# joeyee/Onet

Hardware: AMD Instinct MI355X
Metric: training images/sec (twin 256x256 pass) (higher is better)
Workload: dtype f32

## Files before the change

### onet_amd/csrc/bn.hip

```cpp
#include <type_traits>
#include "common.hpp"

using namespace onet;

__global__ __launch_bounds__(256) void bn_stats_partial_kernel(const float* __restrict__ z, int64_t z_bs,
                                                               float* __restrict__ part, int C, int HW,
                                                               int chunks, int chunk_len) {
    __shared__ double red[16];
    const int c = blockIdx.x % C;
    const int p = blockIdx.x / C;
    const int b = p / chunks, ch = p % chunks;
    const float* src = z + (int64_t)b * z_bs + (int64_t)c * HW;
    const int beg = ch * chunk_len;
    const int end = min(beg + chunk_len, HW);
    const bool vec = ((HW & 3) == 0) && ((z_bs & 3) == 0) && ((chunk_len & 3) == 0);
    const double pivot = (double)src[beg];
    double v[2] = {0.0, 0.0};
    if (vec) {
        int i = beg + threadIdx.x * 4;
        for (; i + 3072 < end; i += 4096) {
            float4 q[4];
#pragma unroll
            for (int k = 0; k < 4; ++k) q[k] = *reinterpret_cast<const float4*>(src + i + 1024 * k);
#pragma unroll
// ... 563 lines not shown
    const float* ds = da + (int64_t)b * da_bs + (int64_t)c * HW;
    const int beg = ch * chunk_len, end = min(beg + chunk_len, HW);
    double v[2] = {0.0, 0.0};
    if (((HW & 3) == 0) && ((z_bs & 3) == 0) && ((da_bs & 3) == 0) && ((chunk_len & 3) == 0)) {
        int i = beg + threadIdx.x * 4;
        for (; i + 3072 < end; i += 4096) {
            float4 q[4], g[4];
#pragma unroll
            for (int k = 0; k < 4; ++k) {
                q[k] = bn_ldz4<ZT>(zs + i + 1024 * k);
                g[k] = *reinterpret_cast<const float4*>(ds + i + 1024 * k);
            }
#pragma unroll
            for (int k = 0; k < 4; ++k) {
                const float zz[4] = {q[k].x, q[k].y, q[k].z, q[k].w}, gg[4] = {g[k].x, g[k].y, g[k].z, g[k].w};
#pragma unroll
                for (int e = 0; e < 4; ++e) {
                    const double dy = fmaf(zz[e] - mean, sc, sh) > 0.f ? (double)gg[e] : 0.0;
                    v[0] += dy;
                    v[1] += dy * (((double)zz[e] - meand) * invd);
                    vmax = fmaxf(vmax, fabsf(gg[e]));
                }
            }
        }
        for (; i < end; i += 1024) {
            const float4 q = bn_ldz4<ZT>(zs + i);
            const float4 g = *reinterpret_cast<const float4*>(ds + i);
            const float zz[4] = {q.x, q.y, q.z, q.w}, gg[4] = {g.x, g.y, g.z, g.w};
#pragma unroll
            for (int k = 0; k < 4; ++k) {
                const double dy = fmaf(zz[k] - mean, sc, sh) > 0.f ? (double)gg[k] : 0.0;
                v[0] += dy;
                v[1] += dy * (((double)zz[k] - meand) * invd);
                vmax = fmaxf(vmax, fabsf(gg[k]));
            }
        }
    } else {
        for (int i = beg + threadIdx.x; i < end; i += 256) {
            const float zi = bn_ldz<ZT>(zs + i);
            const double dy = fmaf(zi - mean, sc, sh) > 0.f ? (double)ds[i] : 0.0;
            v[0] += dy;
            v[1] += dy * (((double)zi - meand) * invd);
            vmax = fmaxf(vmax, fabsf(ds[i]));
        }
    }
    amax_commit(vmax, amax);
    block_sum_256<double, 2>(v, red);
    if (threadIdx.x == 0) {
        float* o = part2 + ((int64_t)p * C + c) * 4;
        o[0] = (float)v[0];
        o[1] = (float)(v[0] - (double)o[0]);
        o[2] = (float)v[1];
        o[3] = (float)(v[1] - (double)o[2]);
    }
}

__global__ __launch_bounds__(256) void head_bwd_reduce_kernel(const float* __restrict__ L, int64_t L_bs, const float* __restrict__ z,
                                                              int64_t z_bs, const float* __restrict__ g, const float* __restrict__ at_t,
                                                              const float* __restrict__ at_d, const float* __restrict__ save,
                                                              float* __restrict__ dL, float* __restrict__ part2, int C, int HW, int chunks,
                                                              int chunk_len, unsigned* __restrict__ amax, int gimg) {
    __shared__ double red[8];
    float vmax = 0.f;
    const int c = blockIdx.x % C;
    const int p = blockIdx.x / C;
    const int b = p / chunks, ch = p % chunks;
    save += (int64_t)(b / gimg) * 4 * C;
    const float mean = save[c], invstd = save[C + c], sc = save[2 * C + c], sh = save[3 * C + c];
    const double meand = mean, invd = invstd;
    const float* zs = z + (int64_t)b * z_bs + (int64_t)c * HW;
    const float* ls = L + (int64_t)b * L_bs + (int64_t)c * HW;
    const float* gs = g + (int64_t)b * HW;
    const float* as = b < gimg ? at_t : at_d;
    if (as) as += (int64_t)(b % gimg) * HW;
    float* os = dL + ((int64_t)b * C + c) * HW;
    const int beg = ch * chunk_len, end = min(beg + chunk_len, HW);
    const float4 zero4 = make_float4(0.f, 0.f, 0.f, 0.f);
    double v[2] = {0.0, 0.0};
    auto four = [&](const float4& q, const float4& l, const float4& gv, const float4& av) -> float4 {
        const float zz[4] = {q.x, q.y, q.z, q.w}, ll[4] = {l.x, l.y, l.z, l.w}, gg[4] = {gv.x, gv.y, gv.z, gv.w}, aa[4] = {av.x, av.y, av.z, av.w};
        float o[4];
#pragma unroll
        for (int e = 0; e < 4; ++e) {
            const float x = fmaf(zz[e] - mean, sc, sh);
            o[e] = fmaf(gg[e], fmaxf(x, 0.f), aa[e]);
            const float da = gg[e] * ll[e];
            const double dy = x > 0.f ? (double)da : 0.0;
            v[0] += dy;
            v[1] += dy * (((double)zz[e] - meand) * invd);
            vmax = fmaxf(vmax, fabsf(da));
        }
        return make_float4(o[0], o[1], o[2], o[3]);
    };
    int i = beg + threadIdx.x * 4;
    for (; i + 3072 < end; i += 4096) {
        float4 q[4], l[4], gv[4], av[4];
#pragma unroll
        for (int k = 0; k < 4; ++k) {
            q[k] = *reinterpret_cast<const float4*>(zs + i + 1024 * k);
            l[k] = *reinterpret_cast<const float4*>(ls + i + 1024 * k);
            gv[k] = *reinterpret_cast<const float4*>(gs + i + 1024 * k);
            av[k] = as ? *reinterpret_cast<const float4*>(as + i + 1024 * k) : zero4;
        }
#pragma unroll
        for (int k = 0; k < 4; ++k) *reinterpret_cast<float4*>(os + i + 1024 * k) = four(q[k], l[k], gv[k], av[k]);
    }
// ... 197 lines not shown
}

int onet_bn_finalize_cm(const float* part, int nparts, int64_t c_stride, const float* gamma, const float* beta, float* running_mean,
                            float* running_var, float momentum, float eps, float* save, void* act_amax, int groups, int C, void* stream) {
    ONET_REQUIRE(part && save && nparts > 0 && C > 0 && groups >= 1 && c_stride >= (int64_t)nparts * groups * 3, "bn_finalize_cm: bad args");
    hipLaunchKernelGGL(bn_finalize_cm_kernel, dim3(C), dim3(256), 0, as_stream(stream), part, nparts, c_stride, gamma, beta, running_mean,
                       running_var, momentum, eps, save, C, (unsigned*)act_amax, groups);
    return check_launch("bn_finalize_cm_kernel");
}

int onet_bn_eval_coeffs(const float* gamma, const float* beta, const float* running_mean,
                        const float* running_var, float eps, float* save, int C, void* stream) {
    ONET_REQUIRE(running_mean && running_var && save && C > 0, "bn_eval_coeffs: bad args");
    hipLaunchKernelGGL(bn_eval_coeffs_kernel, dim3(cdiv(C, 256)), dim3(256), 0, as_stream(stream), gamma, beta,
                       running_mean, running_var, eps, save, C);
    return check_launch("bn_eval_coeffs_kernel");
}

int onet_bn_relu_apply(const void* z, int z_bf16, int64_t z_bs, float* a, int64_t a_bs, const float* save, void* amax, int group_images,
                            int B, int C, int HW, void* stream) {
    ONET_REQUIRE(z && a && save && B > 0 && C > 0 && HW > 0 && group_images >= 0, "bn_relu_apply: bad args");
    const int chunks = cdiv(HW, 4096);
    const int64_t blocks = (int64_t)B * C * chunks;
    ONET_REQUIRE(blocks < (1ll << 31), "bn_relu_apply: grid too large");
    if (z_bf16) {
        ONET_REQUIRE((reinterpret_cast<uintptr_t>(z) & 7) == 0, "bn_relu_apply: 8-byte aligned bf16 rows required");
        hipLaunchKernelGGL(bn_relu_apply_kernel<__bf16>, dim3((unsigned)blocks), dim3(256), 0, as_stream(stream), (const __bf16*)z, z_bs, a, a_bs,
                           save, C, HW, chunks, (unsigned*)amax, group_images);
    } else {
        hipLaunchKernelGGL(bn_relu_apply_kernel<float>, dim3((unsigned)blocks), dim3(256), 0, as_stream(stream), (const float*)z, z_bs, a, a_bs,
                           save, C, HW, chunks, (unsigned*)amax, group_images);
    }
    return check_launch("bn_relu_apply_kernel");
}

int onet_bn_relu_apply_pool(const float* z, int64_t z_bs, float* a, int64_t a_bs, float* y, int64_t y_bs, const float* save,
                                 void* amax, int B, int C, int H, int W, void* stream) {
    ONET_REQUIRE(z && a && y && save && B > 0 && C > 0 && H > 0 && W > 0, "bn_relu_apply_pool: bad args");
    auto al = [](const void* p, uintptr_t m) { return (reinterpret_cast<uintptr_t>(p) & m) == 0; };
    if ((H & 1) || (W & 3) || (z_bs & 3) || (a_bs & 3) || (y_bs & 1) || !al(z, 15) || !al(a, 15) || !al(y, 7)) return 1;
    const int npatch = (H / 2) * (W / 4), bpp = cdiv(npatch, 256);
    const int64_t blocks = (int64_t)B * C * bpp;
    ONET_REQUIRE(blocks < (1ll << 31), "bn_relu_apply_pool: grid too large");
    hipLaunchKernelGGL(bn_relu_apply_pool_kernel, dim3((unsigned)blocks), dim3(256), 0, as_stream(stream), z, z_bs, a, a_bs,
                       y, y_bs, save, C, H, W, bpp, (unsigned*)amax);
    return check_launch("bn_relu_apply_pool_kernel");
}

int onet_bn_relu_bwd_reduce(const float* da, int64_t da_bs, const void* z, int z_bf16, int64_t z_bs, const float* save, float* part2,
                                 int nparts, void* da_amax, int group_images, int B, int C, int HW, void* stream) {
    ONET_REQUIRE(da && z && save && part2 && B > 0 && C > 0 && HW > 0 && group_images >= 0, "bn_relu_bwd_reduce: bad args");
    int chunks, chunk_len;
    ONET_REQUIRE(split_plan(nparts, B, HW, chunks, chunk_len), "bn_relu_bwd_reduce: nparts=%d must be a multiple of B=%d that leaves no chunk of HW=%d empty", nparts, B, HW);
    const dim3 grid((unsigned)((int64_t)nparts * C));
    if (z_bf16) {
        ONET_REQUIRE((reinterpret_cast<uintptr_t>(z) & 7) == 0, "bn_relu_bwd_reduce: 8-byte aligned bf16 rows required");
        hipLaunchKernelGGL(bn_relu_bwd_reduce_kernel<__bf16>, grid, dim3(256), 0, as_stream(stream), da, da_bs, (const __bf16*)z, z_bs, save,
                           part2, C, HW, chunks, chunk_len, (unsigned*)da_amax, group_images);
    } else {
        hipLaunchKernelGGL(bn_relu_bwd_reduce_kernel<float>, grid, dim3(256), 0, as_stream(stream), da, da_bs, (const float*)z, z_bs, save,
                           part2, C, HW, chunks, chunk_len, (unsigned*)da_amax, group_images);
    }
    return check_launch("bn_relu_bwd_reduce_kernel");
}

int onet_bn_bwd_bound(const float* save, const float* coef, const void* da_amax, int64_t count, void* dz_amax, int C, void* stream) {
    ONET_REQUIRE(save && da_amax && dz_amax && count > 0 && C > 0, "bn_bwd_bound: bad args");
    hipLaunchKernelGGL(bn_bwd_bound_kernel, dim3(cdiv(C, 64)), dim3(64), 0, as_stream(stream), save, coef, (const unsigned*)da_amax,
                       sqrtf((float)(count > 1 ? count - 1 : 1)), (unsigned*)dz_amax, C);
    return check_launch("bn_bwd_bound_kernel");
}

int onet_bn_relu_apply_split(const void* z, int z_bf16, int64_t z_bs, void* xs, int64_t xs_bs, float* a, int64_t a_bs, const float* save,
                             const void* act_amax, int nparts, int group_images, int B, int C, int H, int W, void* stream) {
    ONET_REQUIRE(nparts == 1 || nparts == 2, "bn_relu_apply_split: nparts must be 2 (fp16 hi | mid) or 1 (plain bf16)");
    ONET_REQUIRE(z && xs && save && B > 0 && C > 0 && (C % 8) == 0 && H > 0 && W > 0 && (W % 4) == 0, "bn_relu_apply_split: bad args (C %% 8 == 0, W %% 4 == 0)");
    ONET_REQUIRE((reinterpret_cast<uintptr_t>(xs) & 15) == 0 && (xs_bs & 3) == 0 && (reinterpret_cast<uintptr_t>(z) & 15) == 0 && (z_bs & 3) == 0 &&
                 (reinterpret_cast<uintptr_t>(a) & 15) == 0 && (a_bs & 3) == 0, "bn_relu_apply_split: 16-byte aligned rows and slots required");
    const int bpp = cdiv((int64_t)H * W, 1024);
    const int64_t blocks = (int64_t)B * (C / 8) * bpp;
    ONET_REQUIRE(blocks < (1ll << 31) && (int64_t)H * W < (1 << 24), "bn_relu_apply_split: grid too large");
    if (z_bf16)
        hipLaunchKernelGGL(bn_relu_apply_split_kernel<__bf16>, dim3((unsigned)blocks), dim3(256), bn_tr_bytes(nparts), as_stream(stream), (const __bf16*)z, z_bs,
                           (unsigned*)xs, xs_bs, a, a_bs, save, C, H, W, bpp, nparts, (const unsigned*)act_amax, group_images);
    else
        hipLaunchKernelGGL(bn_relu_apply_split_kernel<float>, dim3((unsigned)blocks), dim3(256), bn_tr_bytes(nparts), as_stream(stream), (const float*)z, z_bs,
                           (unsigned*)xs, xs_bs, a, a_bs, save, C, H, W, bpp, nparts, (const unsigned*)act_amax, group_images);
    return check_launch("bn_relu_apply_split_kernel");
}

int onet_bn_relu_apply_pool_split(const void* z, int z_bf16, int64_t z_bs, void* xs, int64_t xs_bs, float* a, int64_t a_bs, void* ys, int64_t ys_bs,
                                  float* y, int64_t y_bs, const float* save, const void* act_amax, int nparts, int group_images, int B, int C,
                                  int H, int W, void* stream) {
    ONET_REQUIRE(nparts == 1 || nparts == 2, "bn_relu_apply_pool_split: nparts must be 2 (fp16 hi | mid) or 1 (plain bf16)");
    ONET_REQUIRE(z && (xs || a) && (ys || y) && save && B > 0 && C > 0 && (C % 8) == 0 && H > 0 && W > 0, "bn_relu_apply_pool_split: bad args");
    auto al = [](const void* p, uintptr_t m) { return (reinterpret_cast<uintptr_t>(p) & m) == 0; };
    if ((H & 1) || (W & 3) || (z_bs & 3) || (a_bs & 3) || (xs_bs & 3) || (ys_bs & 3) || (y_bs & 1) || !al(z, 15) || !al(a, 15) || !al(xs, 15) ||
        !al(ys, 15) || !al(y, 7))
        return 1;
    const int bpp = cdiv((int64_t)(H / 2) * (W / 4), 256);
    const int64_t blocks = (int64_t)B * (C / 8) * bpp;
    ONET_REQUIRE(blocks < (1ll << 31) && (int64_t)H * W < (1 << 24), "bn_relu_apply_pool_split: grid too large");
    if (z_bf16)
        hipLaunchKernelGGL(bn_relu_apply_pool_split_kernel<__bf16>, dim3((unsigned)blocks), dim3(256), bn_tr_bytes(nparts), as_stream(stream), (const __bf16*)z, z_bs,
                           (unsigned*)xs, xs_bs, a, a_bs, (unsigned*)ys, ys_bs, y, y_bs, save, C, H, W, bpp, nparts, (const unsigned*)act_amax,
                           group_images);
    else
        hipLaunchKernelGGL(bn_relu_apply_pool_split_kernel<float>, dim3((unsigned)blocks), dim3(256), bn_tr_bytes(nparts), as_stream(stream), (const float*)z, z_bs,
                           (unsigned*)xs, xs_bs, a, a_bs, (unsigned*)ys, ys_bs, y, y_bs, save, C, H, W, bpp, nparts, (const unsigned*)act_amax,
// ... 84 lines not shown
```

### onet_amd/csrc/spatial.hip

```cpp
#include "common.hpp"

using namespace onet;

static inline unsigned grid_for(int64_t n, int per_block = 256) {
    int64_t b = (n + per_block - 1) / per_block;
    if (b > 16384) b = 16384;
    if (b < 1) b = 1;
    return (unsigned)b;
}

__global__ void maxpool2_fwd_kernel(const float* __restrict__ x, int64_t x_bs, float* __restrict__ y,
                                    int64_t y_bs, int B, int C, int H, int W, int Ho, int Wo) {
    const int64_t n = (int64_t)B * C * Ho * Wo;
    for (int64_t i = blockIdx.x * (int64_t)blockDim.x + threadIdx.x; i < n; i += (int64_t)gridDim.x * blockDim.x) {
        const int ox = (int)(i % Wo);
        int64_t r = i / Wo;
        const int oy = (int)(r % Ho);
        r /= Ho;
        const int c = (int)(r % C), b = (int)(r / C);
        const float* p = x + (int64_t)b * x_bs + (int64_t)c * H * W + (int64_t)(2 * oy) * W + 2 * ox;
        const float2 t = *reinterpret_cast<const float2*>(p);
        const float2 u = *reinterpret_cast<const float2*>(p + W);
        const float m = fmaxf(fmaxf(t.x, t.y), fmaxf(u.x, u.y));
        y[(int64_t)b * y_bs + (int64_t)c * Ho * Wo + (int64_t)oy * Wo + ox] = m;
// ... 240 lines not shown

__global__ void bilinear2x_bwd_kernel(const float* __restrict__ dy, int64_t dy_bs, float* __restrict__ dx,
                                      int64_t dx_bs, int B, int C, int h, int w, int Ho, int Wo, int pt, int pl) {
    const int64_t n = (int64_t)B * C * h * w;
    for (int64_t i = blockIdx.x * (int64_t)blockDim.x + threadIdx.x; i < n; i += (int64_t)gridDim.x * blockDim.x) {
        const int ix = (int)(i % w);
        int64_t r = i / w;
        const int iy = (int)(r % h);
        r /= h;
        const int c = (int)(r % C), b = (int)(r / C);
        float wy[BIL_MAXC], wx[BIL_MAXC];
        int ylo, xlo;
        const int ny = bil_candidates(iy, h, 2 * h, ylo, wy), nx = bil_candidates(ix, w, 2 * w, xlo, wx);
        const float* g = dy + (int64_t)b * dy_bs + (int64_t)c * Ho * Wo + (int64_t)(ylo + pt) * Wo + xlo + pl;
        float acc = 0.f;
        for (int ky = 0; ky < ny; ++ky) {
            float row = 0.f;
            for (int kx = 0; kx < nx; ++kx) row = fmaf(wx[kx], g[(int64_t)ky * Wo + kx], row);
            acc = fmaf(wy[ky], row, acc);
        }
        dx[(int64_t)b * dx_bs + (int64_t)c * h * w + (int64_t)iy * w + ix] = acc;
    }
}

__global__ void complement_clip_kernel(const float* __restrict__ x, float* __restrict__ y, float bias, int64_t n) {
    for (int64_t i = blockIdx.x * (int64_t)blockDim.x + threadIdx.x; i < n; i += (int64_t)gridDim.x * blockDim.x)
        y[i] = fminf(fmaxf(1.f - x[i] + bias, 0.f), 1.f);
}

__global__ void fill_kernel(float* __restrict__ p, float v, int64_t n) {
    for (int64_t i = blockIdx.x * (int64_t)blockDim.x + threadIdx.x; i < n; i += (int64_t)gridDim.x * blockDim.x) p[i] = v;
}

__global__ void axpy_kernel(const float* __restrict__ x, int64_t x_bs, float* __restrict__ y, int64_t y_bs, float a,
                            int B, int64_t n, int accumulate) {
    const int64_t tot = (int64_t)B * n;
    for (int64_t i = blockIdx.x * (int64_t)blockDim.x + threadIdx.x; i < tot; i += (int64_t)gridDim.x * blockDim.x) {
        const int b = (int)(i / n);
        const int64_t j = i % n;
        float* o = y + (int64_t)b * y_bs + j;
        const float v = a * x[(int64_t)b * x_bs + j];
        *o = accumulate ? *o + v : v;
    }
}


template <typename ZT> __device__ __forceinline__ float4 pool_ldz4(const ZT* p);
template <> __device__ __forceinline__ float4 pool_ldz4<float>(const float* p) { return *reinterpret_cast<const float4*>(p); }
template <> __device__ __forceinline__ float4 pool_ldz4<__bf16>(const __bf16* p) {
    const uint2 u = *reinterpret_cast<const uint2*>(p);
    return make_float4(__builtin_bit_cast(float, u.x << 16), __builtin_bit_cast(float, u.x & 0xffff0000u),
                       __builtin_bit_cast(float, u.y << 16), __builtin_bit_cast(float, u.y & 0xffff0000u));
}
template <typename ZT = float>
__global__ __launch_bounds__(256) void maxpool2_bwd_bn_kernel(const float* __restrict__ x, int64_t x_bs,
                                                              const float* __restrict__ dy, int64_t dy_bs,
                                                              const float* __restrict__ add, int64_t add_bs,
                                                              const float* __restrict__ add2, int64_t add2_bs,
                                                              float* __restrict__ dx, int64_t dx_bs,
                                                              const ZT* __restrict__ z, int64_t z_bs,
                                                              const float* __restrict__ save, int group_images,
                                                              float* __restrict__ part2, int C, int H, int W, int bands,
                                                              int band_rows, unsigned* __restrict__ amax = nullptr) {
    __shared__ double red[8];
    float vmax = 0.f;
    const int c = blockIdx.x % C, p = blockIdx.x / C;
    const int b = p / bands, band = p % bands;
    const int Ho = H >> 1, Wo = W >> 1, W4 = W >> 2;
    const float* sv = save + (int64_t)(b / group_images) * 4 * C;
    const float mean = sv[c], invstd = sv[C + c], sc = sv[2 * C + c], sh = sv[3 * C + c];
    const double meand = mean, invd = invstd;
    const int oy0 = band * (band_rows >> 1), oy1 = min(oy0 + (band_rows >> 1), Ho);
    const int npatch = (oy1 - oy0) * W4;
    double v[2] = {0.0, 0.0};
    for (int i = threadIdx.x; i < npatch; i += 256) {
        const int q = i % W4, oy = oy0 + i / W4;
        const int64_t in_off = (int64_t)c * H * W + (int64_t)(2 * oy) * W + 4 * q;
        const float4 z0 = pool_ldz4<ZT>(z + (int64_t)b * z_bs + in_off);
        const float4 z1 = pool_ldz4<ZT>(z + (int64_t)b * z_bs + in_off + W);
        float4 r0, r1;
        if (x) {
            r0 = *reinterpret_cast<const float4*>(x + (int64_t)b * x_bs + in_off);
            r1 = *reinterpret_cast<const float4*>(x + (int64_t)b * x_bs + in_off + W);
        } else {
            r0 = make_float4(fmaxf(fmaf(z0.x - mean, sc, sh), 0.f), fmaxf(fmaf(z0.y - mean, sc, sh), 0.f),
                             fmaxf(fmaf(z0.z - mean, sc, sh), 0.f), fmaxf(fmaf(z0.w - mean, sc, sh), 0.f));
            r1 = make_float4(fmaxf(fmaf(z1.x - mean, sc, sh), 0.f), fmaxf(fmaf(z1.y - mean, sc, sh), 0.f),
                             fmaxf(fmaf(z1.z - mean, sc, sh), 0.f), fmaxf(fmaf(z1.w - mean, sc, sh), 0.f));
        }
        const float2 g = *reinterpret_cast<const float2*>(dy + (int64_t)b * dy_bs + (int64_t)c * Ho * Wo + (int64_t)oy * Wo + 2 * q);
        int a0 = 0, a1 = 0;
        float m0 = r0.x, m1 = r0.z;
        if (r0.y > m0) { m0 = r0.y; a0 = 1; }
        if (r1.x > m0) { m0 = r1.x; a0 = 2; }
        if (r1.y > m0) { m0 = r1.y; a0 = 3; }
        if (r0.w > m1) { m1 = r0.w; a1 = 1; }
        if (r1.z > m1) { m1 = r1.z; a1 = 2; }
        if (r1.w > m1) { m1 = r1.w; a1 = 3; }
        float o[8] = {a0 == 0 ? g.x : 0.f, a0 == 1 ? g.x : 0.f, a1 == 0 ? g.y : 0.f, a1 == 1 ? g.y : 0.f,
                      a0 == 2 ? g.x : 0.f, a0 == 3 ? g.x : 0.f, a1 == 2 ? g.y : 0.f, a1 == 3 ? g.y : 0.f};
        if (add) {
            const float4 p0 = *reinterpret_cast<const float4*>(add + (int64_t)b * add_bs + in_off);
            const float4 p1 = *reinterpret_cast<const float4*>(add + (int64_t)b * add_bs + in_off + W);
            o[0] += p0.x; o[1] += p0.y; o[2] += p0.z; o[3] += p0.w; o[4] += p1.x; o[5] += p1.y; o[6] += p1.z; o[7] += p1.w;
        }
        if (add2) {
            const float4 p0 = *reinterpret_cast<const float4*>(add2 + (int64_t)b * add2_bs + in_off);
            const float4 p1 = *reinterpret_cast<const float4*>(add2 + (int64_t)b * add2_bs + in_off + W);
            o[0] += p0.x; o[1] += p0.y; o[2] += p0.z; o[3] += p0.w; o[4] += p1.x; o[5] += p1.y; o[6] += p1.z; o[7] += p1.w;
        }
        float* dst = dx + (int64_t)b * dx_bs + in_off;
        *reinterpret_cast<float4*>(dst) = make_float4(o[0], o[1], o[2], o[3]);
        *reinterpret_cast<float4*>(dst + W) = make_float4(o[4], o[5], o[6], o[7]);
        const float zz[8] = {z0.x, z0.y, z0.z, z0.w, z1.x, z1.y, z1.z, z1.w};
#pragma unroll
        for (int k = 0; k < 8; ++k) {
            const double dyk = fmaf(zz[k] - mean, sc, sh) > 0.f ? (double)o[k] : 0.0;
            v[0] += dyk;
            v[1] += dyk * (((double)zz[k] - meand) * invd);
            vmax = fmaxf(vmax, fabsf(o[k]));
        }
    }
    if (amax) {
        __shared__ float wmax[4];
#pragma unroll
        for (int o = 32; o > 0; o >>= 1) vmax = fmaxf(vmax, __shfl_xor(vmax, o, 64));
        if ((threadIdx.x & 63) == 0) wmax[threadIdx.x >> 6] = vmax;
        __syncthreads();
        if (threadIdx.x == 0) {
            const float m = fmaxf(fmaxf(wmax[0], wmax[1]), fmaxf(wmax[2], wmax[3]));
            unsigned* sl = amax + (blockIdx.x & 63) * 32;
            const unsigned bits = __builtin_bit_cast(unsigned, m);
            if (m == m && __builtin_nontemporal_load(sl) < bits) atomicMax(sl, bits);
        }
    }
    block_sum_256<double, 2>(v, red);
    if (threadIdx.x == 0) {
        float* o = part2 + ((int64_t)p * C + c) * 4;
        o[0] = (float)v[0];
        o[1] = (float)(v[0] - (double)o[0]);
        o[2] = (float)v[1];
        o[3] = (float)(v[1] - (double)o[2]);
    }
}

static void pool_bn_plan(int H, int W, int& bands, int& band_rows) {
    band_rows = std::max(2, (16384 / std::max(W, 1)) & ~1);
    bands = cdiv(H, band_rows);
}

static int maxpool2_bwd_impl(const float* x, int64_t x_bs, const float* dy, int64_t dy_bs, float* dx, int64_t dx_bs, int B,
                             int C, int H, int W, int accumulate, const float* add, int64_t add_bs, const float* add2,
                             int64_t add2_bs, void* stream) {
    const int64_t n = (int64_t)B * C * H * W;
    const bool v4 = ((W & 3) == 0) && ((H & 1) == 0) && ((x_bs & 3) == 0) && ((dx_bs & 3) == 0) && ((dy_bs & 1) == 0) &&
                    ((add_bs & 3) == 0) && ((reinterpret_cast<uintptr_t>(add) & 15) == 0) &&
                    ((add2_bs & 3) == 0) && ((reinterpret_cast<uintptr_t>(add2) & 15) == 0) &&
                    ((reinterpret_cast<uintptr_t>(x) & 15) == 0) && ((reinterpret_cast<uintptr_t>(dx) & 15) == 0) &&
                    ((reinterpret_cast<uintptr_t>(dy) & 7) == 0);
    if (v4) {
        hipLaunchKernelGGL(maxpool2_bwd_v4_kernel, dim3(grid_for(n / 8)), dim3(256), 0, as_stream(stream), x, x_bs, dy, dy_bs,
                           dx, dx_bs, B, C, H, W, accumulate, add, add_bs, add2, add2_bs);
        return check_launch("maxpool2_bwd_v4_kernel");
    }
    hipLaunchKernelGGL(maxpool2_bwd_kernel, dim3(grid_for(n)), dim3(256), 0, as_stream(stream), x, x_bs, dy, dy_bs, dx,
                       dx_bs, B, C, H, W, H / 2, W / 2, accumulate, add, add_bs, add2, add2_bs);
    return check_launch("maxpool2_bwd_kernel");
}

extern "C" {

int onet_maxpool2_fwd(const float* x, int64_t x_bs, float* y, int64_t y_bs, int B, int C, int H, int W,
                      void* stream) {
    ONET_REQUIRE(x && y && B > 0 && C > 0 && H >= 2 && W >= 2, "maxpool2_fwd: bad args (H=%d W=%d)", H, W);
    const int Ho = H / 2, Wo = W / 2;
    const int64_t n = (int64_t)B * C * Ho * Wo;
    const bool aligned = ((W & 1) == 0) && ((x_bs & 1) == 0) && ((reinterpret_cast<uintptr_t>(x) & 7) == 0);
    if (aligned)
        hipLaunchKernelGGL(maxpool2_fwd_kernel, dim3(grid_for(n)), dim3(256), 0, as_stream(stream), x, x_bs, y, y_bs, B, C, H, W, Ho, Wo);
    else
        hipLaunchKernelGGL(maxpool2_fwd_kernel_s, dim3(grid_for(n)), dim3(256), 0, as_stream(stream), x, x_bs, y, y_bs, B, C, H, W, Ho, Wo);
    return check_launch("maxpool2_fwd_kernel");
}

int onet_maxpool2_bwd(const float* x, int64_t x_bs, const float* dy, int64_t dy_bs, const float* add, int64_t add_bs,
                      const float* add2, int64_t add2_bs, float* dx, int64_t dx_bs, int B, int C, int H, int W, int accumulate,
                      void* stream) {
    ONET_REQUIRE(x && dy && dx && (add || !add2) && !(add && accumulate) && B > 0 && C > 0 && H >= 2 && W >= 2, "maxpool2_bwd: bad args");
    return maxpool2_bwd_impl(x, x_bs, dy, dy_bs, dx, dx_bs, B, C, H, W, accumulate, add, add_bs, add2, add2_bs, stream);
}

int onet_maxpool2_bwd_bn_bands(int H, int W) {
    if (H < 2 || W < 4 || (W & 3) || (H & 1)) return 0;
    int bands, rows;
    pool_bn_plan(H, W, bands, rows);
    return bands;
}

static int maxpool2_bwd_add_bnreduce_impl(const float* x, int64_t x_bs, const float* dy, int64_t dy_bs, const float* add, int64_t add_bs,
                                          const float* add2, int64_t add2_bs, float* dx, int64_t dx_bs, const void* z, int z_bf16, int64_t z_bs,
                                          const float* save, int group_images, float* part2, unsigned* amax, int B, int C, int H, int W,
                                          void* stream);

int onet_maxpool2_bwd_add_bnreduce(const float* x, int64_t x_bs, const float* dy, int64_t dy_bs, const float* add, int64_t add_bs,
                                        const float* add2, int64_t add2_bs, float* dx, int64_t dx_bs, const void* z, int z_bf16, int64_t z_bs,
                                        const float* save, int group_images, float* part2, void* dx_amax, int B, int C, int H, int W,
                                        void* stream) {
    return maxpool2_bwd_add_bnreduce_impl(x, x_bs, dy, dy_bs, add, add_bs, add2, add2_bs, dx, dx_bs, z, z_bf16, z_bs, save, group_images, part2,
                                          (unsigned*)dx_amax, B, C, H, W, stream);
}

static int maxpool2_bwd_add_bnreduce_impl(const float* x, int64_t x_bs, const float* dy, int64_t dy_bs, const float* add, int64_t add_bs,
                                          const float* add2, int64_t add2_bs, float* dx, int64_t dx_bs, const void* z, int z_bf16, int64_t z_bs,
                                          const float* save, int group_images, float* part2, unsigned* amax, int B, int C, int H, int W,
                                          void* stream) {
    ONET_REQUIRE(dy && dx && z && save && part2 && B > 0 && C > 0, "maxpool2_bwd_add_bnreduce: bad args");
    ONET_REQUIRE(group_images > 0 && (B % group_images) == 0, "maxpool2_bwd_add_bnreduce: bad statistics groups");
    const bool ok = H >= 2 && W >= 4 && ((W & 3) == 0) && ((H & 1) == 0) && ((x_bs & 3) == 0) && ((dx_bs & 3) == 0) &&
                    ((z_bs & 3) == 0) && ((dy_bs & 1) == 0) && ((add_bs & 3) == 0) && ((add2_bs & 3) == 0) &&
                    ((reinterpret_cast<uintptr_t>(x) & 15) == 0) && ((reinterpret_cast<uintptr_t>(dx) & 15) == 0) &&
                    ((reinterpret_cast<uintptr_t>(z) & 15) == 0) && ((reinterpret_cast<uintptr_t>(add) & 15) == 0) &&
                    ((reinterpret_cast<uintptr_t>(add2) & 15) == 0) && ((reinterpret_cast<uintptr_t>(dy) & 7) == 0);
    ONET_REQUIRE(ok, "maxpool2_bwd_add_bnreduce: W %% 4 == 0, even H and 16-byte aligned planes required (onet_maxpool2_bwd_bn_bands() == 0 elsewhere)");
    int bands, rows;
    pool_bn_plan(H, W, bands, rows);
    const int64_t blocks = (int64_t)B * bands * C;
    ONET_REQUIRE(blocks < (1ll << 31), "maxpool2_bwd_add_bnreduce: grid too large");
    if (z_bf16)
        hipLaunchKernelGGL(maxpool2_bwd_bn_kernel<__bf16>, dim3((unsigned)blocks), dim3(256), 0, as_stream(stream), x, x_bs, dy, dy_bs, add,
                           add_bs, add2, add2_bs, dx, dx_bs, (const __bf16*)z, z_bs, save, group_images, part2, C, H, W, bands, rows, amax);
    else
        hipLaunchKernelGGL(maxpool2_bwd_bn_kernel<float>, dim3((unsigned)blocks), dim3(256), 0, as_stream(stream), x, x_bs, dy, dy_bs, add,
                           add_bs, add2, add2_bs, dx, dx_bs, (const float*)z, z_bs, save, group_images, part2, C, H, W, bands, rows, amax);
    return check_launch("maxpool2_bwd_bn_kernel");
}

int onet_pixel_shuffle2_bias(const float* sub, const float* bias, float* y, int64_t y_bs, int B, int C, int h,
                             int w, int Ho, int Wo, int pt, int pl, void* stream) {
    ONET_REQUIRE(sub && y && B > 0 && C > 0 && h > 0 && w > 0, "pixel_shuffle2: bad args");
    ONET_REQUIRE(pt >= 0 && pl >= 0 && pt + 2 * h <= Ho && pl + 2 * w <= Wo, "pixel_shuffle2: window outside plane");
    const int64_t n = (int64_t)B * C * Ho * Wo;
    hipLaunchKernelGGL(pixel_shuffle2_bias_kernel, dim3(grid_for(n)), dim3(256), 0, as_stream(stream), sub, bias, y,
                       y_bs, B, C, h, w, Ho, Wo, pt, pl);
    return check_launch("pixel_shuffle2_bias_kernel");
}

int onet_copy_strided(const float* src, int64_t src_bs, float* dst, int64_t dst_bs, int B, int64_t n,
                      void* stream) {
    ONET_REQUIRE(src && dst && B > 0 && n > 0, "copy_strided: bad args");
    const bool v4 = ((n & 3) == 0) && ((src_bs & 3) == 0) && ((dst_bs & 3) == 0) &&
                    ((reinterpret_cast<uintptr_t>(src) & 15) == 0) && ((reinterpret_cast<uintptr_t>(dst) & 15) == 0);
    if (v4)
        hipLaunchKernelGGL(copy_strided_kernel, dim3(grid_for((int64_t)B * n / 4)), dim3(256), 0, as_stream(stream), src, src_bs, dst, dst_bs, B, n / 4);
    else
        hipLaunchKernelGGL(copy_strided_kernel_s, dim3(grid_for((int64_t)B * n)), dim3(256), 0, as_stream(stream), src, src_bs, dst, dst_bs, B, n);
    return check_launch("copy_strided_kernel");
}

int onet_bilinear2x_fwd(const float* x, int64_t x_bs, float* y, int64_t y_bs, int B, int C, int h, int w, int Ho,
                        int Wo, int pt, int pl, void* stream) {
    ONET_REQUIRE(x && y && B > 0 && C > 0 && h > 0 && w > 0, "bilinear2x_fwd: bad args");
    ONET_REQUIRE(pt >= 0 && pl >= 0 && pt + 2 * h <= Ho && pl + 2 * w <= Wo, "bilinear2x_fwd: window outside plane");
    const int64_t n = (int64_t)B * C * Ho * Wo;
    hipLaunchKernelGGL(bilinear2x_fwd_kernel, dim3(grid_for(n)), dim3(256), 0, as_stream(stream), x, x_bs, y, y_bs, B, C,
                       h, w, Ho, Wo, pt, pl);
    return check_launch("bilinear2x_fwd_kernel");
}

int onet_complement_clip(const float* x, float* y, float bias, int64_t n, void* stream) {
    ONET_REQUIRE(x && y && n > 0, "complement_clip: bad args");
    hipLaunchKernelGGL(complement_clip_kernel, dim3(grid_for(n)), dim3(256), 0, as_stream(stream), x, y, bias, n);
    return check_launch("complement_clip_kernel");
}

int onet_fill(float* p, float value, int64_t n, void* stream) {
    ONET_REQUIRE(p && n > 0, "fill: bad args");
    hipLaunchKernelGGL(fill_kernel, dim3(grid_for(n)), dim3(256), 0, as_stream(stream), p, value, n);
    return check_launch("fill_kernel");
}

int onet_axpy(const float* x, int64_t x_bs, float* y, int64_t y_bs, float a, int B, int64_t n, int accumulate,
              void* stream) {
    ONET_REQUIRE(x && y && B > 0 && n > 0, "axpy: bad args");
    hipLaunchKernelGGL(axpy_kernel, dim3(grid_for((int64_t)B * n)), dim3(256), 0, as_stream(stream), x, x_bs, y, y_bs, a, B, n, accumulate);
    return check_launch("axpy_kernel");
}
// ... 49 lines not shown
```

Measured before the change: 593.6.

## Map small BN backward reductions to single waves instead of full blocks

Adds a wave-per-record variant of the BN-ReLU backward reduction for short chunks, where each 64-lane wave handles one (or a fraction of a) channel chunk and reduces with wave shuffles instead of block-wide shared-memory sums. The maxpool backward + BN reduce kernel is templated to also run one record per wave when bands are small, and gains a LEAN variant that processes two patches per iteration when x and add2 are absent, for more loads in flight. The aim is to cut idle threads and __syncthreads overhead on deep, low-resolution layers. The cost is more template instantiations and register pressure from the double-patch path.

```diff
diff --git a/onet_amd/csrc/bn.hip b/onet_amd/csrc/bn.hip
--- a/onet_amd/csrc/bn.hip
+++ b/onet_amd/csrc/bn.hip
@@ -639,6 +639,72 @@
         o[1] = (float)(v[0] - (double)o[0]);
         o[2] = (float)v[1];
         o[3] = (float)(v[1] - (double)o[2]);
+    }
+}
+
+constexpr int BN_REDUCE_WAVE_LEN = 1024;
+template <typename ZT = float>
+__global__ __launch_bounds__(256) void bn_relu_bwd_reduce_wave_kernel(const float* __restrict__ da, int64_t da_bs,
+                                                                      const ZT* __restrict__ z, int64_t z_bs,
+                                                                      const float* __restrict__ save, float* __restrict__ part2, int C,
+                                                                      int HW, int chunks, int chunk_len, int nrec,
+                                                                      unsigned* __restrict__ amax, int gimg) {
+    const int lane = threadIdx.x & 63;
+    const int lt = chunk_len <= 256 ? 0 : chunk_len <= 512 ? 1 : 2;
+    const int64_t rec0 = ((int64_t)blockIdx.x * 4 + __builtin_amdgcn_readfirstlane((int)(threadIdx.x >> 6))) * (4 >> lt);
+    if (rec0 >= nrec) return;
+    float4 q[4], g[4];
+    float mean[4], invstd[4], sc[4], sh[4];
+    bool live[4];
+#pragma unroll
+    for (int k = 0; k < 4; ++k) {
+        const int rec = (int)min(rec0 + (k >> lt), (int64_t)nrec - 1), trip = k & ((1 << lt) - 1);
+        const int c = rec % C, p = rec / C, b = p / chunks, ch = p % chunks;
+        const float* sv = save + (gimg ? (int64_t)(b / gimg) * 4 * C : 0);
+        mean[k] = sv[c], invstd[k] = sv[C + c], sc[k] = sv[2 * C + c], sh[k] = sv[3 * C + c];
+        const int beg = ch * chunk_len, end = min(beg + chunk_len, HW), i = beg + trip * 256 + lane * 4;
+        live[k] = rec0 + (k >> lt) < nrec && i < end;
+        q[k] = make_float4(0.f, 0.f, 0.f, 0.f), g[k] = q[k];
+        if (live[k]) {
+            q[k] = bn_ldz4<ZT>(z + (int64_t)b * z_bs + (int64_t)c * HW + i);
+            g[k] = *reinterpret_cast<const float4*>(da + (int64_t)b * da_bs + (int64_t)c * HW + i);
+        }
+    }
+    double v[2] = {0.0, 0.0};
+    float vmax = 0.f;
+#pragma unroll
+    for (int k = 0; k < 4; ++k) {
+        if ((k & ((1 << lt) - 1)) == 0) v[0] = 0.0, v[1] = 0.0, vmax = 0.f;
+        if (live[k]) {
+            const double meand = mean[k], invd = invstd[k];
+            const float zz[4] = {q[k].x, q[k].y, q[k].z, q[k].w}, gg[4] = {g[k].x, g[k].y, g[k].z, g[k].w};
+#pragma unroll
+            for (int e = 0; e < 4; ++e) {
+                const double dy = fmaf(zz[e] - mean[k], sc[k], sh[k]) > 0.f ? (double)gg[e] : 0.0;
+                v[0] += dy;
+                v[1] += dy * (((double)zz[e] - meand) * invd);
+                vmax = fmaxf(vmax, fabsf(gg[e]));
+            }
+        }
+        const int64_t rec = rec0 + (k >> lt);
+        if (((k + 1) & ((1 << lt) - 1)) == 0 && rec < nrec) {
+            const double s0 = wave_sum(v[0]), s1 = wave_sum(v[1]);
+            float m = vmax;
+#pragma unroll
+            for (int o = 32; o > 0; o >>= 1) m = fmaxf(m, __shfl_xor(m, o, 64));
+            if (lane == 0) {
+                float* o = part2 + rec * 4;
+                o[0] = (float)s0;
+                o[1] = (float)(s0 - (double)o[0]);
+                o[2] = (float)s1;
+                o[3] = (float)(s1 - (double)o[2]);
+                if (amax && m == m) {
+                    unsigned* s = amax + (int)(rec & 63) * AMAX_STRIDE;
+                    const unsigned bits = __builtin_bit_cast(unsigned, m);
+                    if (__builtin_nontemporal_load(s) < bits) atomicMax(s, bits);
+                }
+            }
+        }
     }
 }
 
@@ -942,9 +1008,22 @@
     ONET_REQUIRE(da && z && save && part2 && B > 0 && C > 0 && HW > 0 && group_images >= 0, "bn_relu_bwd_reduce: bad args");
     int chunks, chunk_len;
     ONET_REQUIRE(split_plan(nparts, B, HW, chunks, chunk_len), "bn_relu_bwd_reduce: nparts=%d must be a multiple of B=%d that leaves no chunk of HW=%d empty", nparts, B, HW);
-    const dim3 grid((unsigned)((int64_t)nparts * C));
+    const int64_t nrec = (int64_t)nparts * C;
+    ONET_REQUIRE(nrec < (1ll << 31), "bn_relu_bwd_reduce: grid too large");
+    if (z_bf16) ONET_REQUIRE((reinterpret_cast<uintptr_t>(z) & 7) == 0, "bn_relu_bwd_reduce: 8-byte aligned bf16 rows required");
+    if (chunk_len <= BN_REDUCE_WAVE_LEN && (HW & 3) == 0 && (z_bs & 3) == 0 && (da_bs & 3) == 0) {
+        const int per_block = 4 * (chunk_len <= 256 ? 4 : chunk_len <= 512 ? 2 : 1);
+        const dim3 wgrid((unsigned)((nrec + per_block - 1) / per_block));
+        if (z_bf16)
+            hipLaunchKernelGGL(bn_relu_bwd_reduce_wave_kernel<__bf16>, wgrid, dim3(256), 0, as_stream(stream), da, da_bs, (const __bf16*)z, z_bs,
+                               save, part2, C, HW, chunks, chunk_len, (int)nrec, (unsigned*)da_amax, group_images);
+        else
+            hipLaunchKernelGGL(bn_relu_bwd_reduce_wave_kernel<float>, wgrid, dim3(256), 0, as_stream(stream), da, da_bs, (const float*)z, z_bs,
+                               save, part2, C, HW, chunks, chunk_len, (int)nrec, (unsigned*)da_amax, group_images);
+        return check_launch("bn_relu_bwd_reduce_wave_kernel");
+    }
+    const dim3 grid((unsigned)nrec);
     if (z_bf16) {
-        ONET_REQUIRE((reinterpret_cast<uintptr_t>(z) & 7) == 0, "bn_relu_bwd_reduce: 8-byte aligned bf16 rows required");
         hipLaunchKernelGGL(bn_relu_bwd_reduce_kernel<__bf16>, grid, dim3(256), 0, as_stream(stream), da, da_bs, (const __bf16*)z, z_bs, save,
                            part2, C, HW, chunks, chunk_len, (unsigned*)da_amax, group_images);
     } else {
diff --git a/onet_amd/csrc/spatial.hip b/onet_amd/csrc/spatial.hip
--- a/onet_amd/csrc/spatial.hip
+++ b/onet_amd/csrc/spatial.hip
@@ -316,7 +316,73 @@
     return make_float4(__builtin_bit_cast(float, u.x << 16), __builtin_bit_cast(float, u.x & 0xffff0000u),
                        __builtin_bit_cast(float, u.y << 16), __builtin_bit_cast(float, u.y & 0xffff0000u));
 }
-template <typename ZT = float>
+struct PoolPatch {
+    float4 z0, z1, r0, r1, p0, p1, q0, q1;
+    float2 g;
+};
+template <typename ZT>
+__device__ __forceinline__ void pool_patch_load(PoolPatch& t, const ZT* __restrict__ z, const float* __restrict__ x, const float* __restrict__ dy,
+                                                const float* __restrict__ add, const float* __restrict__ add2, int64_t in_off, int64_t g_off, int W) {
+    t.z0 = pool_ldz4<ZT>(z + in_off);
+    t.z1 = pool_ldz4<ZT>(z + in_off + W);
+    if (x) {
+        t.r0 = *reinterpret_cast<const float4*>(x + in_off);
+        t.r1 = *reinterpret_cast<const float4*>(x + in_off + W);
+    }
+    t.g = *reinterpret_cast<const float2*>(dy + g_off);
+    if (add) {
+        t.p0 = *reinterpret_cast<const float4*>(add + in_off);
+        t.p1 = *reinterpret_cast<const float4*>(add + in_off + W);
+    }
+    if (add2) {
+        t.q0 = *reinterpret_cast<const float4*>(add2 + in_off);
+        t.q1 = *reinterpret_cast<const float4*>(add2 + in_off + W);
+    }
+}
+__device__ __forceinline__ void pool_patch_step(const PoolPatch& t, bool has_x, bool has_add, bool has_add2, float* __restrict__ dst, int W,
+                                                float mean, float sc, float sh, double meand, double invd, double (&v)[2], float& vmax) {
+    const float4 z0 = t.z0, z1 = t.z1;
+    float4 r0, r1;
+    if (has_x) {
+        r0 = t.r0;
+        r1 = t.r1;
+    } else {
+        r0 = make_float4(fmaxf(fmaf(z0.x - mean, sc, sh), 0.f), fmaxf(fmaf(z0.y - mean, sc, sh), 0.f),
+                         fmaxf(fmaf(z0.z - mean, sc, sh), 0.f), fmaxf(fmaf(z0.w - mean, sc, sh), 0.f));
+        r1 = make_float4(fmaxf(fmaf(z1.x - mean, sc, sh), 0.f), fmaxf(fmaf(z1.y - mean, sc, sh), 0.f),
+                         fmaxf(fmaf(z1.z - mean, sc, sh), 0.f), fmaxf(fmaf(z1.w - mean, sc, sh), 0.f));
+    }
+    const float2 g = t.g;
+    int a0 = 0, a1 = 0;
+    float m0 = r0.x, m1 = r0.z;
+    if (r0.y > m0) { m0 = r0.y; a0 = 1; }
+    if (r1.x > m0) { m0 = r1.x; a0 = 2; }
+    if (r1.y > m0) { m0 = r1.y; a0 = 3; }
+    if (r0.w > m1) { m1 = r0.w; a1 = 1; }
+    if (r1.z > m1) { m1 = r1.z; a1 = 2; }
+    if (r1.w > m1) { m1 = r1.w; a1 = 3; }
+    float o[8] = {a0 == 0 ? g.x : 0.f, a0 == 1 ? g.x : 0.f, a1 == 0 ? g.y : 0.f, a1 == 1 ? g.y : 0.f,
+                  a0 == 2 ? g.x : 0.f, a0 == 3 ? g.x : 0.f, a1 == 2 ? g.y : 0.f, a1 == 3 ? g.y : 0.f};
+    if (has_add) {
+        const float4 p0 = t.p0, p1 = t.p1;
+        o[0] += p0.x; o[1] += p0.y; o[2] += p0.z; o[3] += p0.w; o[4] += p1.x; o[5] += p1.y; o[6] += p1.z; o[7] += p1.w;
+    }
+    if (has_add2) {
+        const float4 p0 = t.q0, p1 = t.q1;
+        o[0] += p0.x; o[1] += p0.y; o[2] += p0.z; o[3] += p0.w; o[4] += p1.x; o[5] += p1.y; o[6] += p1.z; o[7] += p1.w;
+    }
+    *reinterpret_cast<float4*>(dst) = make_float4(o[0], o[1], o[2], o[3]);
+    *reinterpret_cast<float4*>(dst + W) = make_float4(o[4], o[5], o[6], o[7]);
+    const float zz[8] = {z0.x, z0.y, z0.z, z0.w, z1.x, z1.y, z1.z, z1.w};
+#pragma unroll
+    for (int k = 0; k < 8; ++k) {
+        const double dyk = fmaf(zz[k] - mean, sc, sh) > 0.f ? (double)o[k] : 0.0;
+        v[0] += dyk;
+        v[1] += dyk * (((double)zz[k] - meand) * invd);
+        vmax = fmaxf(vmax, fabsf(o[k]));
+    }
+}
+template <typename ZT = float, int G = 256, bool LEAN = false>
 __global__ __launch_bounds__(256) void maxpool2_bwd_bn_kernel(const float* __restrict__ x, int64_t x_bs,
                                                               const float* __restrict__ dy, int64_t dy_bs,
                                                               const float* __restrict__ add, int64_t add_bs,
@@ -325,10 +391,14 @@
                                                               const ZT* __restrict__ z, int64_t z_bs,
                                                               const float* __restrict__ save, int group_images,
                                                               float* __restrict__ part2, int C, int H, int W, int bands,
-                                                              int band_rows, unsigned* __restrict__ amax = nullptr) {
-    __shared__ double red[8];
+                                                              int band_rows, int nrec, unsigned* __restrict__ amax = nullptr) {
+    static_assert(G == 256 || G == 64, "a record belongs to a block or to a wave");
+    if constexpr (LEAN) x = nullptr, add2 = nullptr;
     float vmax = 0.f;
-    const int c = blockIdx.x % C, p = blockIdx.x / C;
+    const int rec = G == 256 ? (int)blockIdx.x : (int)blockIdx.x * 4 + (int)(threadIdx.x >> 6);
+    const int gt = G == 256 ? (int)threadIdx.x : (int)(threadIdx.x & 63);
+    if (G == 64 && rec >= nrec) return;
+    const int c = rec % C, p = rec / C;
     const int b = p / bands, band = p % bands;
     const int Ho = H >> 1, Wo = W >> 1, W4 = W >> 2;
     const float* sv = save + (int64_t)(b / group_images) * 4 * C;
@@ -336,70 +406,50 @@
     const double meand = mean, invd = invstd;
     const int oy0 = band * (band_rows >> 1), oy1 = min(oy0 + (band_rows >> 1), Ho);
     const int npatch = (oy1 - oy0) * W4;
+    const bool has_x = x != nullptr, has_add = add != nullptr, has_add2 = add2 != nullptr;
+    z += (int64_t)b * z_bs;
+    dx += (int64_t)b * dx_bs;
+    dy += (int64_t)b * dy_bs + (int64_t)c * Ho * Wo;
+    if (has_x) x += (int64_t)b * x_bs;
+    if (has_add) add += (int64_t)b * add_bs;
+    if (has_add2) add2 += (int64_t)b * add2_bs;
+    const int64_t plane = (int64_t)c * H * W;
     double v[2] = {0.0, 0.0};
-    for (int i = threadIdx.x; i < npatch; i += 256) {
-        const int q = i % W4, oy = oy0 + i / W4;
-        const int64_t in_off = (int64_t)c * H * W + (int64_t)(2 * oy) * W + 4 * q;
-        const float4 z0 = pool_ldz4<ZT>(z + (int64_t)b * z_bs + in_off);
-        const float4 z1 = pool_ldz4<ZT>(z + (int64_t)b * z_bs + in_off + W);
-        float4 r0, r1;
-        if (x) {
-            r0 = *reinterpret_cast<const float4*>(x + (int64_t)b * x_bs + in_off);
-            r1 = *reinterpret_cast<const float4*>(x + (int64_t)b * x_bs + in_off + W);
-        } else {
-            r0 = make_float4(fmaxf(fmaf(z0.x - mean, sc, sh), 0.f), fmaxf(fmaf(z0.y - mean, sc, sh), 0.f),
-                             fmaxf(fmaf(z0.z - mean, sc, sh), 0.f), fmaxf(fmaf(z0.w - mean, sc, sh), 0.f));
-            r1 = make_float4(fmaxf(fmaf(z1.x - mean, sc, sh), 0.f), fmaxf(fmaf(z1.y - mean, sc, sh), 0.f),
-                             fmaxf(fmaf(z1.z - mean, sc, sh), 0.f), fmaxf(fmaf(z1.w - mean, sc, sh), 0.f));
-        }
-        const float2 g = *reinterpret_cast<const float2*>(dy + (int64_t)b * dy_bs + (int64_t)c * Ho * Wo + (int64_t)oy * Wo + 2 * q);
-        int a0 = 0, a1 = 0;
-        float m0 = r0.x, m1 = r0.z;
-        if (r0.y > m0) { m0 = r0.y; a0 = 1; }
-        if (r1.x > m0) { m0 = r1.x; a0 = 2; }
-        if (r1.y > m0) { m0 = r1.y; a0 = 3; }
-        if (r0.w > m1) { m1 = r0.w; a1 = 1; }
-        if (r1.z > m1) { m1 = r1.z; a1 = 2; }
-        if (r1.w > m1) { m1 = r1.w; a1 = 3; }
-        float o[8] = {a0 == 0 ? g.x : 0.f, a0 == 1 ? g.x : 0.f, a1 == 0 ? g.y : 0.f, a1 == 1 ? g.y : 0.f,
-                      a0 == 2 ? g.x : 0.f, a0 == 3 ? g.x : 0.f, a1 == 2 ? g.y : 0.f, a1 == 3 ? g.y : 0.f};
-        if (add) {
-            const float4 p0 = *reinterpret_cast<const float4*>(add + (int64_t)b * add_bs + in_off);
-            const float4 p1 = *reinterpret_cast<const float4*>(add + (int64_t)b * add_bs + in_off + W);
-            o[0] += p0.x; o[1] += p0.y; o[2] += p0.z; o[3] += p0.w; o[4] += p1.x; o[5] += p1.y; o[6] += p1.z; o[7] += p1.w;
-        }
-        if (add2) {
-            const float4 p0 = *reinterpret_cast<const float4*>(add2 + (int64_t)b * add2_bs + in_off);
-            const float4 p1 = *reinterpret_cast<const float4*>(add2 + (int64_t)b * add2_bs + in_off + W);
-            o[0] += p0.x; o[1] += p0.y; o[2] += p0.z; o[3] += p0.w; o[4] += p1.x; o[5] += p1.y; o[6] += p1.z; o[7] += p1.w;
-        }
-        float* dst = dx + (int64_t)b * dx_bs + in_off;
-        *reinterpret_cast<float4*>(dst) = make_float4(o[0], o[1], o[2], o[3]);
-        *reinterpret_cast<float4*>(dst + W) = make_float4(o[4], o[5], o[6], o[7]);
-        const float zz[8] = {z0.x, z0.y, z0.z, z0.w, z1.x, z1.y, z1.z, z1.w};
-#pragma unroll
-        for (int k = 0; k < 8; ++k) {
-            const double dyk = fmaf(zz[k] - mean, sc, sh) > 0.f ? (double)o[k] : 0.0;
-            v[0] += dyk;
-            v[1] += dyk * (((double)zz[k] - meand) * invd);
-            vmax = fmaxf(vmax, fabsf(o[k]));
-        }
+    constexpr int NP = LEAN ? 2 : 1;
+    for (int i = gt; i < npatch; i += NP * G) {
+        const int i1 = i + G;
+        const bool two = NP == 2 && i1 < npatch;
+        const int q0 = i % W4, y0 = oy0 + i / W4, q1 = i1 % W4, y1 = oy0 + i1 / W4;
+        const int64_t off0 = plane + (int64_t)(2 * y0) * W + 4 * q0, off1 = plane + (int64_t)(2 * y1) * W + 4 * q1;
+        PoolPatch t0, t1;
+        pool_patch_load<ZT>(t0, z, x, dy, add, add2, off0, (int64_t)y0 * Wo + 2 * q0, W);
+        if (two) pool_patch_load<ZT>(t1, z, x, dy, add, add2, off1, (int64_t)y1 * Wo + 2 * q1, W);
+        pool_patch_step(t0, has_x, has_add, has_add2, dx + off0, W, mean, sc, sh, meand, invd, v, vmax);
+        if (two) pool_patch_step(t1, has_x, has_add, has_add2, dx + off1, W, mean, sc, sh, meand, invd, v, vmax);
     }
     if (amax) {
-        __shared__ float wmax[4];
 #pragma unroll
         for (int o = 32; o > 0; o >>= 1) vmax = fmaxf(vmax, __shfl_xor(vmax, o, 64));
-        if ((threadIdx.x & 63) == 0) wmax[threadIdx.x >> 6] = vmax;
-        __syncthreads();
-        if (threadIdx.x == 0) {
-            const float m = fmaxf(fmaxf(wmax[0], wmax[1]), fmaxf(wmax[2], wmax[3]));
-            unsigned* sl = amax + (blockIdx.x & 63) * 32;
-            const unsigned bits = __builtin_bit_cast(unsigned, m);
-            if (m == m && __builtin_nontemporal_load(sl) < bits) atomicMax(sl, bits);
-        }
-    }
-    block_sum_256<double, 2>(v, red);
-    if (threadIdx.x == 0) {
+        if constexpr (G == 256) {
+            __shared__ float wmax[4];
+            if ((threadIdx.x & 63) == 0) wmax[threadIdx.x >> 6] = vmax;
+            __syncthreads();
+            vmax = fmaxf(fmaxf(wmax[0], wmax[1]), fmaxf(wmax[2], wmax[3]));
+        }
+        if (gt == 0) {
+            unsigned* sl = amax + (rec & 63) * 32;
+            const unsigned bits = __builtin_bit_cast(unsigned, vmax);
+            if (vmax == vmax && __builtin_nontemporal_load(sl) < bits) atomicMax(sl, bits);
+        }
+    }
+    if constexpr (G == 256) {
+        __shared__ double red[8];
+        block_sum_256<double, 2>(v, red);
+    } else {
+        v[0] = wave_sum(v[0]);
+        v[1] = wave_sum(v[1]);
+    }
+    if (gt == 0) {
         float* o = part2 + ((int64_t)p * C + c) * 4;
         o[0] = (float)v[0];
         o[1] = (float)(v[0] - (double)o[0]);
@@ -408,6 +458,7 @@
     }
 }
 
+constexpr int POOL_BN_WAVE_PATCHES = 256;
 static void pool_bn_plan(int H, int W, int& bands, int& band_rows) {
     band_rows = std::max(2, (16384 / std::max(W, 1)) & ~1);
     bands = cdiv(H, band_rows);
@@ -488,14 +539,28 @@
     ONET_REQUIRE(ok, "maxpool2_bwd_add_bnreduce: W %% 4 == 0, even H and 16-byte aligned planes required (onet_maxpool2_bwd_bn_bands() == 0 elsewhere)");
     int bands, rows;
     pool_bn_plan(H, W, bands, rows);
-    const int64_t blocks = (int64_t)B * bands * C;
-    ONET_REQUIRE(blocks < (1ll << 31), "maxpool2_bwd_add_bnreduce: grid too large");
-    if (z_bf16)
-        hipLaunchKernelGGL(maxpool2_bwd_bn_kernel<__bf16>, dim3((unsigned)blocks), dim3(256), 0, as_stream(stream), x, x_bs, dy, dy_bs, add,
-                           add_bs, add2, add2_bs, dx, dx_bs, (const __bf16*)z, z_bs, save, group_images, part2, C, H, W, bands, rows, amax);
-    else
-        hipLaunchKernelGGL(maxpool2_bwd_bn_kernel<float>, dim3((unsigned)blocks), dim3(256), 0, as_stream(stream), x, x_bs, dy, dy_bs, add,
-                           add_bs, add2, add2_bs, dx, dx_bs, (const float*)z, z_bs, save, group_images, part2, C, H, W, bands, rows, amax);
+    const int64_t nrec = (int64_t)B * bands * C;
+    ONET_REQUIRE(nrec < (1ll << 31), "maxpool2_bwd_add_bnreduce: grid too large");
+    const bool wave = (std::min(rows, H) >> 1) * (W >> 2) < POOL_BN_WAVE_PATCHES;
+    const dim3 grid((unsigned)(wave ? (nrec + 3) / 4 : nrec));
+#define ONET_POOL_BN_LAUNCH(ZT, G, LEAN)                                                                                                  \
+    hipLaunchKernelGGL((maxpool2_bwd_bn_kernel<ZT, G, LEAN>), grid, dim3(256), 0, as_stream(stream), x, x_bs, dy, dy_bs, add, add_bs,    \
+                       add2, add2_bs, dx, dx_bs, (const ZT*)z, z_bs, save, group_images, part2, C, H, W, bands, rows, (int)nrec, amax)
+#define ONET_POOL_BN_LAUNCH_G(ZT, G)                 \
+    do {                                             \
+        if (lean) ONET_POOL_BN_LAUNCH(ZT, G, true);  \
+        else ONET_POOL_BN_LAUNCH(ZT, G, false);      \
+    } while (0)
+    const bool lean = !x && !add2;
+    if (z_bf16) {
+        if (wave) ONET_POOL_BN_LAUNCH_G(__bf16, 64);
+        else ONET_POOL_BN_LAUNCH_G(__bf16, 256);
+    } else {
+        if (wave) ONET_POOL_BN_LAUNCH_G(float, 64);
+        else ONET_POOL_BN_LAUNCH_G(float, 256);
+    }
+#undef ONET_POOL_BN_LAUNCH_G
+#undef ONET_POOL_BN_LAUNCH
     return check_launch("maxpool2_bwd_bn_kernel");
 }
 
```

Result: no change. 596.7, median of 6 (+0.5%).
